# Darkbblue/generic-diffusion-feature

Measured on AMD Instinct MI355X. Metric: images/sec feature-extract, SDXL 1024^2 single-timestep, higher is better.
Workload: dtype f16; 1 GPU; SDXL UNet 1024x1024 (latent 128x128), batch 16/GPU, t=100, hooks=config_xl_practical (4 ids, 15.73 MB/img), full forward; global_batch=16, parallelism=dp1 (batch sharded, weights broadcast once), residual_stream=fp32 master + fp16 shadow, launched_by=single process, max_inflight_forwards=0

## Files before the change

generic-diffusion-feature_amd/csrc/gemm.hip:

```cpp
#include "gemm_mainloop_ring.h"
#include "gemm_mainloop_8phase.h"
#include "gemm_epilogue.h"
#include <cstdio>
#include <cstdlib>
#include <cstring>
#include <deque>
#include <mutex>
#include <string>

namespace gdf {

template <int MODE, int BM, int BN, int STAGES, bool GEGLU, bool DIT, bool BF = false, bool QKN = false, bool SPLIT = false, bool MX = false,
          bool GNS = false>
__device__ __forceinline__ void gemm_body(const GemmParams& p) {
  using T = GemmTile<MODE, BM, BN, STAGES, GEGLU, DIT, BF, QKN, SPLIT, MX, GNS>;
  extern __shared__ __attribute__((aligned(16))) char smem[];
  T t(p, smem);
  const int tiles_n = (p.N + BN - 1) / BN;
  const int nblk = ((p.M + BM - 1) / BM) * tiles_n;
  constexpr bool PERSIST = (STAGES == 8);
  int vb = blockIdx.x;
  do {
  t.locate(vb, tiles_n, nblk);
  f32x4 acc[T::FM][T::FN];
#pragma unroll
  for (int i = 0; i < T::FM; ++i)
#pragma unroll
    for (int j = 0; j < T::FN; ++j) acc[i][j] = f32x4{0.f, 0.f, 0.f, 0.f};
  if constexpr (STAGES == 8) gemm_mainloop_8phase_256(t, acc);
  else if constexpr (STAGES == 9) gemm_mainloop_8phase_320(t, acc);
  else gemm_mainloop_ring(t, acc);
  __syncthreads();
  gemm_epilogue(t, acc);
  if constexpr (!PERSIST) break;
  vb += gridDim.x;
  if (vb >= nblk) break;
  asm volatile("s_waitcnt lgkmcnt(0)" ::: "memory");
  __builtin_amdgcn_s_barrier();
  } while (true);
}

template <int MODE, int BM, int BN, int STAGES, bool GEGLU>
__global__ __launch_bounds__(BM * 2, 2) void gemm_kernel(const GemmParams p) {
  gemm_body<MODE, BM, BN, STAGES, GEGLU, false>(p);
}
template <int MODE, int BM, int BN, int STAGES>
__global__ __launch_bounds__(BM * 2, 2) void gemm_gn_kernel(const GemmParams p) {
  gemm_body<MODE, BM, BN, STAGES, false, false, false, false, false, false, true>(p);
}
template <int MODE, int BM, int BN, int STAGES, bool GEGLU>
__global__ __launch_bounds__(BM * 2, 2) void gemm_split_kernel(const GemmParams p) {
  gemm_body<MODE, BM, BN, STAGES, GEGLU, false, false, false, true>(p);
}
template <int BM, int BN, int STAGES, bool BF, bool QKN>
__global__ __launch_bounds__(BM * 2, 2) void gemm_dit_kernel(const GemmParams p) {
  gemm_body<A_DENSE, BM, BN, STAGES, false, true, BF, QKN>(p);
}

template <int BM, int BN, int STAGES, bool BF, bool QKN>
__global__ __launch_bounds__(BM * 2, 2) void gemm_dit_split_kernel(const GemmParams p) {
  gemm_body<A_DENSE, BM, BN, STAGES, false, true, BF, QKN, true>(p);
}

template <int BM, int BN, int STAGES>
__global__ __launch_bounds__(BM * 2, 2) void gemm_mx_kernel(const GemmParams p) {
  gemm_body<A_DENSE, BM, BN, STAGES, false, true, true, false, false, true>(p);
}

static int persist_wgs() {
  static const int off = [] { const char* e = getenv("GDF_PERSIST"); return e && atoi(e) == 0; }();
  if (off) return 1 << 30;
  static std::atomic<int> cus[16];
  int dev = 0;
  if (hipGetDevice(&dev) != hipSuccess || dev < 0 || dev >= 16) return 1 << 30;
  int n = cus[dev].load(std::memory_order_relaxed);
  if (n == 0) {
    if (hipDeviceGetAttribute(&n, hipDeviceAttributeMultiprocessorCount, dev) != hipSuccess || n < 8 || (n & 7)) n = 1 << 30;
    cus[dev].store(n, std::memory_order_relaxed);
  }
  return n;
}

template <int MODE, int BM, int BN, int STAGES, bool GEGLU, bool DIT = false, bool BF = false, bool QKN = false, bool SPLIT = false, bool MX = false,
          bool GNS = false>
static hipError_t launch_t(const GemmParams& p, hipStream_t s) {
  const int tiles_m = (p.M + BM - 1) / BM, tiles_n = (p.N + BN - 1) / BN;
  const int smem = (STAGES >= 8 ? 2 : STAGES) * (BM * 128 + BN * 128);
  static std::atomic<uint64_t> attr_mask{0};
  {
    const void* fn;
    if constexpr (MX) fn = (const void*)gemm_mx_kernel<BM, BN, STAGES>;
    else if constexpr (GNS) fn = (const void*)gemm_gn_kernel<MODE, BM, BN, STAGES>;
    else if constexpr (DIT && SPLIT) fn = (const void*)gemm_dit_split_kernel<BM, BN, STAGES, BF, QKN>;
    else if constexpr (DIT) fn = (const void*)gemm_dit_kernel<BM, BN, STAGES, BF, QKN>;
    else if constexpr (SPLIT) fn = (const void*)gemm_split_kernel<MODE, BM, BN, STAGES, GEGLU>;
    else fn = (const void*)gemm_kernel<MODE, BM, BN, STAGES, GEGLU>;
    const hipError_t e = ensure_dyn_smem(attr_mask, fn, smem);
    if (e != hipSuccess) return e;
  }
  GemmParams q = p;
  q.sb_gm = q.sb_gn = 0;
  if (!p.no_superblock) {
    const int conc = (p.cus > 0 ? p.cus / 8 : 32) * ((BM == 256) ? 1 : 2);
    for (int gn = 4; gn >= 2; gn >>= 1) {
      const int gm = conc / gn;
      if (tiles_n % gn == 0 && tiles_m % gm == 0 && (tiles_m / gm) * (tiles_n / gn) >= 8 && tiles_n > gn) {
        q.sb_gm = gm; q.sb_gn = gn;
        break;
      }
    }
  }
  int gx = tiles_m * tiles_n;
  const int pw = (p.cus > 0 && p.cus < persist_wgs()) ? p.cus : persist_wgs();
  if (STAGES == 8 && gx > pw && !(p.batch > 1)) gx = pw;
  const dim3 grid(gx, (STAGES == 2 && p.splitk > 1) ? p.splitk : p.batch > 1 ? p.batch : 1);
  if constexpr (MX) hipLaunchKernelGGL((gemm_mx_kernel<BM, BN, STAGES>), grid, dim3(BM * 2), smem, s, q);
  else if constexpr (GNS) hipLaunchKernelGGL((gemm_gn_kernel<MODE, BM, BN, STAGES>), grid, dim3(BM * 2), smem, s, q);
  else if constexpr (DIT && SPLIT) hipLaunchKernelGGL((gemm_dit_split_kernel<BM, BN, STAGES, BF, QKN>), grid, dim3(BM * 2), smem, s, q);
  else if constexpr (DIT) hipLaunchKernelGGL((gemm_dit_kernel<BM, BN, STAGES, BF, QKN>), grid, dim3(BM * 2), smem, s, q);
  else if constexpr (SPLIT) hipLaunchKernelGGL((gemm_split_kernel<MODE, BM, BN, STAGES, GEGLU>), grid, dim3(BM * 2), smem, s, q);
  else hipLaunchKernelGGL((gemm_kernel<MODE, BM, BN, STAGES, GEGLU>), grid, dim3(BM * 2), smem, s, q);
  return hipGetLastError();
}

static double round_fill(long tiles, int slots) {
  if (tiles <= 0) return 0.0;
  const long rounds = (tiles + slots - 1) / slots;
  return (double)tiles / (double)(rounds * slots);
}

static int pick_variant_any(const GemmParams& p);
static bool is_split(const GemmParams& p) { return !p.dit && (p.k_w > 0 || p.o16_lo > 0); }
static bool is_dit_split(const GemmParams& p) { return p.dit && (p.k_w > 0 || p.o16_lo > 0); }
static int pick_variant(const GemmParams& p) {
  const int v = pick_variant_any(p);
  if (is_dit_split(p)) return (v == 8256 || v == 1256) ? 8256 : 128;
  if (!is_split(p) || v == 16) return v;
  if (p.geglu) return v == 825 ? 825 : 128;
  if (p.mode == A_CONV_SMALLC) return v == 160 ? 160 : 128;
  return (v == 932 || v == 160) ? v : 128;
}
static int pick_variant_any(const GemmParams& p) {
  const int S1 = p.cus > 0 ? p.cus : 256, S2 = 2 * S1;
  if (p.dit) {
    const long t256 = (long)((p.M + 255) / 256) * ((p.N + 255) / 256);
    if (p.variant == 128 || p.variant == 1256 || p.variant == 2128 || p.variant == 8256) return p.variant;
    if (t256 >= 128 && (long)((p.N + 255) / 256) * 256 <= (long)p.N + p.N / 8) return 8256;
    return (p.N % 128 == 0 && (long)((p.M + 255) / 256) * (p.N / 128) >= 256) ? 2128 : 128;
  }
  if (p.bn == 16) return 16;
  if (p.splitk > 1) {
    static const int force = [] { const char* e = getenv("GDF_SPLITK_TILE"); return e ? atoi(e) : 0; }();
    if (force == 160 && p.N % 160 == 0) return 160;
    if (force == 128 && p.N % 128 == 0) return 128;
    return (p.N % 160 == 0) ? 160 : 128;
  }
  if (p.variant) return p.variant;
  const long tiles256 = (long)((p.M + 255) / 256) * ((p.N + 127) / 128);
  const long tiles320 = (long)((p.M + 255) / 256) * ((p.N + 319) / 320);
  if (p.geglu) {
    const long tm256 = (p.M + 255) / 256, tm128 = (p.M + 127) / 128;
    double best = 0.0; int bv = 128;
    auto cand = [&](int v, double rate, long tiles, int slots) { const double sc = rate * round_fill(tiles, slots); if (sc > best) { best = sc; bv = v; } };
    if (p.N % 256 == 0) cand(825, 1.00, tm256 * (p.N / 256), S1);
    if (p.N % 320 == 0) cand(320, 0.95, tm256 * (p.N / 320), S1);
    cand(256, 0.80, tm256 * ((p.N + 127) / 128), S1);
    cand(128, 0.70, tm128 * ((p.N + 127) / 128), S2);
    return bv;
  }
  if (p.mode != A_DENSE) {
    if (p.N % 320 == 0) {
      const double s932 = 1.00 * round_fill(tiles320, S1), s160 = 0.85 * round_fill((long)((p.M + 127) / 128) * (p.N / 160), S2);
      const double s128 = 0.70 * round_fill((long)((p.M + 127) / 128) * ((p.N + 127) / 128), S2);
      return (s932 >= s160 && s932 >= s128) ? 932 : (s160 >= s128 ? 160 : 128);
    }
    if (p.N % 160 == 0) return 160;
    if (p.N % 256 == 0 && (long)((p.M + 255) / 256) * (p.N / 256) >= 256) return 826;
    return (p.N <= 128 && p.M >= (1 << 20)) ? 256 : 128;
  }
  if (p.res32 && p.K <= 1536 && p.N % 160 == 0 && tiles320 <= S2 &&
      !(p.N % 320 == 0 && p.N >= 640 && p.K >= 640 && tiles320 % S1 == 0)) return 160;
  if (p.N % 320 == 0) {
    const double s932 = 1.00 * round_fill(tiles320, S1), s160 = 0.87 * round_fill((long)((p.M + 127) / 128) * (p.N / 160), S2);
    const double s128 = 0.72 * round_fill((long)((p.M + 127) / 128) * ((p.N + 127) / 128), S2);
    return (s932 >= s160 && s932 >= s128) ? 932 : (s160 >= s128 ? 160 : 128);
  }
  if (p.N % 160 == 0 && p.K >= 1024) return 160;
  if ((long)p.M * p.N >= (1L << 26) && tiles256 >= S2) return 256;
  return 128;
}

bool gemm_qkn_ok(int M, int N, int K) {
  GemmParams g{}; g.M = M; g.N = N; g.K = K; g.dit = 1; g.mode = A_DENSE;
  const int v = pick_variant(g);
  return v == 8256 || v == 1256;
}

const char* gemm_kernel_name(const GemmParams& p) {
  const int v = pick_variant(p);
  int bm = 128, bn = 128, st = 2;
  if (v == 16) bn = 16; else if (v == 160) bn = 160; else if (v == 256) { bm = 256; st = 3; } else if (v == 320) { bm = 256; bn = 320; }
  else if (v == 825) { bm = 256; bn = 256; st = 8; } else if (v == 932) { bm = 256; bn = 320; st = 9; } else if (v == 826) { bm = 256; bn = 256; st = 8; }
  if (p.mode == A_CONV_SMALLC && v != 160) { bm = 128; bn = 128; st = 2; }
  char tmp[64];
  if (p.gn_partial && !p.dit) snprintf(tmp, sizeof tmp, "gemm_gn_kernel<%d, %d, %d, %d>", p.mode, bm, bn, st);
  else if (p.dit && p.mx) snprintf(tmp, sizeof tmp, "gemm_mx_kernel<256, 256, 8>");
  else if (p.dit) snprintf(tmp, sizeof tmp, "%s<%d, %d, %d, %s, %s>", is_dit_split(p) ? "gemm_dit_split_kernel" : "gemm_dit_kernel", v == 128 ? 128 : 256, (v == 1256 || v == 8256) ? 256 : 128, v == 8256 ? 8 : v == 2128 ? 3 : 2, p.bf16 ? "true" : "false", p.qkn_nq ? "true" : "false");
  else snprintf(tmp, sizeof tmp, "%s<%d, %d, %d, %d, %s>", is_split(p) ? "gemm_split_kernel" : "gemm_kernel", p.mode, bm, bn, st, p.geglu ? "true" : "false");
  static std::mutex mu;
  static std::deque<std::string> names;
  std::lock_guard<std::mutex> lk(mu);
  for (const std::string& n : names) if (n == tmp) return n.c_str();
  names.emplace_back(tmp);
  return names.back().c_str();
}

int gemm_gn_slab_rows(const GemmParams& p) {
  if ((p.mode != A_CONV3 && p.mode != A_CONV_SMALLC) || p.dit || p.geglu || p.splitk > 1 || p.batch > 1 || is_split(p) || p.bn == 16) return 0;
  if ((p.M % 64) != 0 || (p.N % 8) != 0) return 0;
  const int v = pick_variant(p);
  if (p.mode == A_CONV_SMALLC) return v != 160 ? 64 : 0;
  if (v == 932) return (p.M % 128) == 0 ? 128 : 0;
  return (v == 128 || v == 160 || v == 256 || v == 826) ? 64 : 0;
}

hipError_t gemm_check(const GemmParams& p) {
  if (p.mode != A_CONV_SMALLC && (p.K % BK) != 0) return hipErrorInvalidValue;
  if (p.mode == A_CONV3 && (p.Cin % BK) != 0) return hipErrorInvalidValue;
  if (p.k_w > 0 && (p.K != 2 * p.k_w || (p.k_w % BK) != 0 || p.mode == A_CONV_SMALLC || (p.dit && !p.bf16) || (p.mode == A_CONV3 && (p.k_w % (9 * BK)) != 0)))
    return hipErrorInvalidValue;
  if (p.o16_lo > 0 && ((p.dit && !p.bf16) || p.bn == 16 || (p.o16_lo % 8) != 0)) return hipErrorInvalidValue;
  if (p.out_f16 && !(p.dit && p.bf16)) return hipErrorInvalidValue;
  const int v = pick_variant(p);
  if (v != 16 && ((p.geglu ? p.N / 2 : p.N) % 8) != 0) return hipErrorInvalidValue;
  if (p.bf16 && !p.dit) return hipErrorInvalidValue;
  if (p.gn_partial) return (gemm_gn_slab_rows(p) == 0 || !p.out16) ? hipErrorInvalidValue : hipSuccess;
  if (p.dit) {
    if (p.mode != A_DENSE || p.geglu || p.batch > 1) return hipErrorInvalidValue;
    if (p.qkn_nq && ((v != 8256 && v != 1256) || (p.qkn_nq % 128) != 0)) return hipErrorInvalidValue;
    if (p.qkn_nq && (p.res32 || p.res16 || p.rowvec || p.aux16 || p.out32)) return hipErrorInvalidValue;
    if (p.mx && (!p.bf16 || p.qkn_nq || is_dit_split(p) || (p.N % 8))) return hipErrorInvalidValue;
    if (!p.mx && is_dit_split(p) && v != 8256 && p.qkn_nq) return hipErrorInvalidValue;
    return hipSuccess;
  }
  if (p.geglu && (p.mode != A_DENSE || (p.N % 32) != 0)) return hipErrorInvalidValue;
  if (v == 16 && (p.mode == A_CONV_SMALLC || (is_split(p) && !p.geglu && p.mode != A_CONV3))) return hipErrorInvalidValue;
  return hipSuccess;
}

bool gemm_variant_ok(const GemmParams& p) {
  if (!p.variant || p.dit || p.mode == A_CONV_SMALLC) return true;
  const int v = pick_variant(p);
  if (p.geglu) return v != 16 && v != 160 && v != 932 && v != 826;
  if (p.mode == A_DENSE) return v != 825 && v != 826;
  return v != 825;
}

hipError_t launch_gemm(const GemmParams& p, hipStream_t s) {
  if (p.M <= 0 || p.N <= 0) return hipSuccess;
// ... 178 lines not shown
```

generic-diffusion-feature_amd/csrc/gemm_epilogue.h:

```cpp
#pragma once
#include "gemm_tile.h"

namespace gdf {

template <class T>
__device__ __forceinline__ void gemm_epilogue(T& t, f32x4 (&acc)[T::FM][T::FN]) {
  GDF_TILE_GEOMETRY(T);
  GDF_TILE_STATE(t);
  _Float16* const out16 = t.out16;
  const float* const e_res32 = QKN ? nullptr : p.res32;
  const float* const e_rowvec = QKN ? nullptr : p.rowvec;
  const _Float16* const e_res16 = QKN ? nullptr : p.res16;
  _Float16* const e_aux16 = QKN ? nullptr : p.aux16;
  float* const e_out32 = QKN ? nullptr : (STAGES == 2 && p.splitk > 1) ? p.out32 + (size_t)blockIdx.y * p.o32_sstride : p.out32;
  static_assert(!GEGLU || (FN % 2 == 0), "GEGLU needs an even number of column fragments per wave");
  constexpr int FNV = GEGLU ? FN / 2 : FN;
  constexpr int WTNV = FNV * 16;
  constexpr int SLD = WTNV + 4;
  constexpr int PR = (FM * FN >= 32) ? 16 : 32;
  constexpr int PASSES = WTM / PR;
  constexpr int FPP = FM / PASSES;
  float* st = (float*)(smem) + wave * (PR * SLD);
  constexpr int OUTW = WTNV;
  constexpr int LPR = OUTW / 8;
  constexpr int RPI = 64 / LPR;
  constexpr int NIT = (PR + RPI - 1) / RPI;
  const bool lane_ok = lane < RPI * LPR;
  const int Nout = GEGLU ? p.N / 2 : p.N;
  const int ocol0 = GEGLU ? (n0 + wn * WTN) / 2 : (n0 + wn * WTN);
  const int lc = (lane % LPR) * 8;
  const int col = ocol0 + lc;
  const int nv = (col < Nout) ? ((Nout - col >= 8) ? 8 : (Nout - col)) : 0;
  const bool full = nv == 8;

  const float a_sc = p.acc_scale != 0.f ? p.acc_scale : 1.0f;
  const float o_sc = p.out16_scale != 0.f ? p.out16_scale : 1.0f;
  float mxc[8];
#pragma unroll
  for (int e = 0; e < 8; ++e) mxc[e] = 1.f;
  if constexpr (MX) {
    if (full && p.mx_colscale) {
      const f32x4 c0 = *(const f32x4*)(p.mx_colscale + col), c1 = *(const f32x4*)(p.mx_colscale + col + 4);
#pragma unroll
      for (int e = 0; e < 4; ++e) { mxc[e] = c0[e]; mxc[4 + e] = c1[e]; }
    }
  }
  float bv[8];
  float bh[FNV], bgt[FNV];
#pragma unroll
  for (int e = 0; e < 8; ++e) bv[e] = 0.f;
#pragma unroll
  for (int j = 0; j < FNV; ++j) { bh[j] = 0.f; bgt[j] = 0.f; }
  if (p.bias) {
    if (GEGLU) {
#pragma unroll
      for (int j = 0; j < FNV; ++j) {
        const int bcol = n0 + wn * WTN + j * 32 + frow;
        if (bcol + 16 < p.N) { bh[j] = p.bias[bcol]; bgt[j] = p.bias[bcol + 16]; }
      }
    } else if (full) {
      const f32x4 a0 = *(const f32x4*)(p.bias + col), a1 = *(const f32x4*)(p.bias + col + 4);
#pragma unroll
      for (int e = 0; e < 4; ++e) { bv[e] = a0[e]; bv[4 + e] = a1[e]; }
    } else if (BN == 16) {
      for (int e = 0; e < nv; ++e) bv[e] = p.bias[col + e];
    }
  }

  constexpr bool RAGGED = (BN == 16);
  const bool rv_in_opnd = e_rowvec && !e_res32;
  auto sample_of = [&](int row) -> int {
    if (DIT && p.rv_seg_rows > 0 && row >= p.rv_seg_rows) return (row - p.rv_seg_rows) / p.rv_rps2;
    if (DIT && p.rv_tok) return row % p.rows_per_sample;
    return row / p.rows_per_sample;
  };
  float gsum[GNS ? 8 : 1], gsq[GNS ? 8 : 1];
#pragma unroll
  for (int e = 0; e < (GNS ? 8 : 1); ++e) gsum[e] = gsq[e] = 0.f;
#pragma unroll
  for (int ps = 0; ps < PASSES; ++ps) {
    f32x4 opnd[NIT][2];
    int rowi[NIT];
    bool okr[NIT];
#pragma unroll
    for (int it = 0; it < NIT; ++it) {
      const int lrp = it * RPI + lane / LPR;
      rowi[it] = m0 + wm * WTM + ps * PR + lrp;
      okr[it] = (RAGGED ? nv > 0 : full) && lane_ok && lrp < PR && rowi[it] < p.M;
      opnd[it][0] = opnd[it][1] = f32x4{0.f, 0.f, 0.f, 0.f};
    }
    if (!RAGGED) {
      if (e_res32) {
#pragma unroll
        for (int it = 0; it < NIT; ++it)
          if (okr[it]) {
            const f32x4* rp = (const f32x4*)(e_res32 + (size_t)rowi[it] * p.ldres + col);
            opnd[it][0] = rp[0]; opnd[it][1] = rp[1];
          }
      } else if (e_rowvec) {
#pragma unroll
        for (int it = 0; it < NIT; ++it)
          if (okr[it]) {
            const f32x4* rv = (const f32x4*)(e_rowvec + (size_t)sample_of(rowi[it]) * p.ldrv + col);
            opnd[it][0] = rv[0]; opnd[it][1] = rv[1];
          }
      } else if (e_res16) {
#pragma unroll
        for (int it = 0; it < NIT; ++it)
          if (okr[it]) opnd[it][0] = *(const f32x4*)(e_res16 + (size_t)rowi[it] * p.ldres + col);
      }
    }
#pragma unroll
    for (int i2 = 0; i2 < FPP; ++i2)
#pragma unroll
      for (int j = 0; j < FNV; ++j)
        if constexpr (GEGLU) {
#pragma unroll
          for (int r = 0; r < 4; r += 2) {
            const f32x2 hh = {acc[ps * FPP + i2][2 * j][r], acc[ps * FPP + i2][2 * j][r + 1]};
            const f32x2 gg = {acc[ps * FPP + i2][2 * j + 1][r], acc[ps * FPP + i2][2 * j + 1][r + 1]};
            const f32x2 x = (hh + bh[j]) * gelu_erf2(gg + bgt[j]);
            st[(i2 * 16 + fk * 4 + r) * SLD + j * 16 + frow] = x[0];
            st[(i2 * 16 + fk * 4 + r + 1) * SLD + j * 16 + frow] = x[1];
          }
        } else {
#pragma unroll
          for (int r = 0; r < 4; ++r) st[(i2 * 16 + fk * 4 + r) * SLD + j * 16 + frow] = acc[ps * FPP + i2][j][r] * a_sc;
        }
    __builtin_amdgcn_wave_barrier();
    float v[NIT][8];
#pragma unroll
    for (int it = 0; it < NIT; ++it) {
      int lr = it * RPI + lane / LPR;
      if (!(lane_ok && lr < PR)) lr = 0;
      const f32x4 x0 = *(const f32x4*)(st + lr * SLD + lc), x1 = *(const f32x4*)(st + lr * SLD + lc + 4);
      if constexpr (MX) {
        const float rs = (okr[it] && p.mx_rowscale) ? p.mx_rowscale[rowi[it]] : 1.f;
#pragma unroll
        for (int e = 0; e < 4; ++e) { v[it][e] = x0[e] * (rs * mxc[e]) + bv[e]; v[it][4 + e] = x1[e] * (rs * mxc[4 + e]) + bv[4 + e]; }
      } else {
#pragma unroll
        for (int e = 0; e < 4; ++e) { v[it][e] = x0[e] + bv[e]; v[it][4 + e] = x1[e] + bv[4 + e]; }
      }
    }
    if (DIT && p.act == 1) {
#pragma unroll
      for (int it = 0; it < NIT; ++it)
#pragma unroll
        for (int e = 0; e < 8; ++e) v[it][e] = gelu_tanh(v[it][e]);
    }
    if constexpr (DIT && WTN == 128 && QKN) {
      if (p.qkn_nq > 0 && ocol0 < 2 * p.qkn_nq) {
        const float* nw = (ocol0 < p.qkn_nq ? p.qkn_wq : p.qkn_wk) + lc;
        const f32x4 w0 = *(const f32x4*)nw, w1 = *(const f32x4*)(nw + 4);
#pragma unroll
        for (int it = 0; it < NIT; ++it) {
          float ss = 0.f;
#pragma unroll
          for (int e = 0; e < 8; ++e) ss += v[it][e] * v[it][e];
#pragma unroll
          for (int off = 8; off > 0; off >>= 1) ss += __shfl_xor(ss, off);
          const float r = rsqrtf(ss * (1.0f / 128.0f) + p.qkn_eps);
          const int row = rowi[it];
          const int pos = (p.qkn_seg_rows > 0 && row >= p.qkn_seg_rows) ? p.qkn_pos1 + (row - p.qkn_seg_rows) % p.qkn_rps2
                                                                        : p.qkn_pos0 + row % p.qkn_rps;
          f32x4 c0 = {1.f, 1.f, 1.f, 1.f}, c1 = c0, s0 = {0.f, 0.f, 0.f, 0.f}, s1 = s0;
          if (okr[it]) {
            const float* cp = p.rope_cos + (size_t)pos * 128 + lc;
            const float* sp = p.rope_sin + (size_t)pos * 128 + lc;
            c0 = *(const f32x4*)cp; c1 = *(const f32x4*)(cp + 4); s0 = *(const f32x4*)sp; s1 = *(const f32x4*)(sp + 4);
          }
          float t[8];
#pragma unroll
          for (int e = 0; e < 4; ++e) { t[e] = v[it][e] * r * w0[e]; t[4 + e] = v[it][4 + e] * r * w1[e]; }
          v[it][0] = t[0] * c0[0] - t[1] * s0[0]; v[it][1] = t[1] * c0[1] + t[0] * s0[1];
          v[it][2] = t[2] * c0[2] - t[3] * s0[2]; v[it][3] = t[3] * c0[3] + t[2] * s0[3];
          v[it][4] = t[4] * c1[0] - t[5] * s1[0]; v[it][5] = t[5] * c1[1] + t[4] * s1[1];
          v[it][6] = t[6] * c1[2] - t[7] * s1[2]; v[it][7] = t[7] * c1[3] + t[6] * s1[3];
        }
      }
    }
    const bool aux_early = DIT && p.rv_mul && e_aux16;
    if (!RAGGED && aux_early) {
#pragma unroll
      for (int it = 0; it < NIT; ++it)
        if (okr[it]) {
          f16x8 hv;
#pragma unroll
          for (int e = 0; e < 8; ++e) hv[e] = hook16<DIT>(v[it][e]);
          *(f16x8*)(e_aux16 + (size_t)rowi[it] * p.ldaux + col) = hv;
        }
    }
    if (!RAGGED) {
      if (rv_in_opnd) {
        if (DIT && p.rv_mul) {
#pragma unroll
          for (int it = 0; it < NIT; ++it)
#pragma unroll
            for (int e = 0; e < 4; ++e) { v[it][e] *= opnd[it][0][e]; v[it][4 + e] *= opnd[it][1][e]; }
        } else {
#pragma unroll
          for (int it = 0; it < NIT; ++it)
#pragma unroll
            for (int e = 0; e < 4; ++e) { v[it][e] += opnd[it][0][e]; v[it][4 + e] += opnd[it][1][e]; }
        }
      } else if (e_rowvec) {
#pragma unroll
        for (int it = 0; it < NIT; ++it)
          if (okr[it]) {
            const f32x4* rv = (const f32x4*)(e_rowvec + (size_t)sample_of(rowi[it]) * p.ldrv + col);
            if (DIT && p.rv_mul) {
#pragma unroll
              for (int e = 0; e < 4; ++e) { v[it][e] *= rv[0][e]; v[it][4 + e] *= rv[1][e]; }
            } else {
#pragma unroll
              for (int e = 0; e < 4; ++e) { v[it][e] += rv[0][e]; v[it][4 + e] += rv[1][e]; }
            }
          }
      }
      if (e_aux16 && !aux_early) {
#pragma unroll
// ... 107 lines not shown
```

generic-diffusion-feature_amd/csrc/gemm_mainloop_8phase.h:

```cpp
#pragma once
#include "gemm_tile.h"

namespace gdf {

template <class T>
__device__ __forceinline__ void gemm_mainloop_8phase_256(T& t, f32x4 (&acc)[T::FM][T::FN]) {
  GDF_TILE_GEOMETRY(T);
  GDF_TILE_STATE(t);
  GDF_TILE_OPERANDS(t);
  static_assert((MODE == A_DENSE || MODE == A_CONV3) && BM == 256 && (BN == 256 || BN == 320) && FM == 4 && FN == BN / 32, "8-phase schedule: 4x2 waves of 64 x BN/2");
  constexpr int FNH = FN / 2;
  constexpr int BHALF = BN / 2;
  constexpr bool B3 = (BN == 320);
  const bool g1 = wave >= 4;
  auto b_unit_row = [&](int unit, int j) { return (wave >> 2) * 128 + unit * 64 + ((wave & 3) * 2 + j) * 8; };
  uint32_t ha[2][2], hb[2][3];
  uint32_t hm[2][2];
  int hbq[2];
#pragma unroll
  for (int h = 0; h < 2; ++h) {
    const bool big = B3 && (g1 == (h == 1));
    hbq[h] = !B3 ? wave * 2 : (big ? (wave & 3) * 3 : 12 + (wave & 3) * 2);
#pragma unroll
    for (int j = 0; j < 2; ++j) {
      const int m = m0 + h * 128 + (wave * 2 + j) * 8 + lrow;
      if (MODE == A_DENSE) {
        ha[h][j] = (m < p.M) ? (uint32_t)m * (uint32_t)p.lda * 2u + (uint32_t)chunk * 16u : OOB;
        hm[h][j] = 0;
      } else {
        conv_row(m, ha[h][j], hm[h][j]);
      }
    }
#pragma unroll
    for (int j = 0; j < 3; ++j) {
      const int r = (B3 ? h * BHALF + (hbq[h] + j) * 8 : b_unit_row(h, j)) + lrow;
      hb[h][j] = (n0 + r < p.N) ? (uint32_t)(n0 + r) * ldb + (uint32_t)chunk * 16u : OOB;
    }
  }
  auto stage = [&](int kt, int buf, auto which) {
    constexpr int W = decltype(which)::value;
    if constexpr (W < 2) {
      char* base = smem + buf * A_TILE + W * 16384 + wave * 2048;
#pragma unroll
      for (int j = 0; j < 2; ++j) {
        glds16(rsA, base + j * 1024, MODE == A_DENSE ? ha[W][j] + koffA(kt) : conv_off(kt, ha[W][j], hm[W][j]));
      }
    } else {
      constexpr int H = W - 2;
      char* base = smem + 2 * A_TILE + buf * B_TILE + (B3 ? H * (BHALF * 128) + hbq[H] * 1024 : b_unit_row(H, 0) * 128);
#pragma unroll
      for (int j = 0; j < 2; ++j) glds16(rsB, base + j * 1024, hb[H][j] + koffB(kt));
      if (B3 && (g1 == (H == 1))) glds16(rsB, base + 2 * 1024, hb[H][2] + koffB(kt));
    }
  };
  auto wait_tile = [&]() {
    if (B3 && !g1) wait_vmcnt<7>(); else wait_vmcnt<6>();
  };
  constexpr std::integral_constant<int, 0> ALO{};
  constexpr std::integral_constant<int, 1> AHI{};
  constexpr std::integral_constant<int, 2> BLO{};
  constexpr std::integral_constant<int, 3> BHI{};
  f16x8 a8[4][2], b8[FNH][2];
  uint32_t fa[2], fb[2];
#pragma unroll
  for (int kk = 0; kk < 2; ++kk) {
    const int ch = MX ? 2 * fk + kk : kk * 4 + fk;
    fa[kk] = (uint32_t)((wm * WTM + frow) * 128 + ((ch ^ (frow & 7)) << 4));
    fb[kk] = (uint32_t)(2 * A_TILE + (wn * WTN + frow) * 128 + ((ch ^ (frow & 7)) << 4));
    asm volatile("" : "+v"(fa[kk]), "+v"(fb[kk]));
  }
  auto rd_a = [&](const int cur) {
#pragma unroll
    for (int i = 0; i < 4; ++i)
#pragma unroll
      for (int kk = 0; kk < 2; ++kk) a8[i][kk] = *(const f16x8*)(smem + fa[kk] + (cur * A_TILE + i * 2048));
  };
  auto rd_b = [&](const int cur, int half) {
#pragma unroll
    for (int j = 0; j < FNH; ++j)
#pragma unroll
      for (int kk = 0; kk < 2; ++kk) b8[j][kk] = *(const f16x8*)(smem + fb[kk] + (cur * B_TILE + (half * FNH + j) * 2048));
  };
  auto mma_q = [&](auto ah, auto bh) {
    constexpr int AH = decltype(ah)::value, BH = decltype(bh)::value;
    if constexpr (MX) {
#pragma unroll
      for (int i = 0; i < 2; ++i)
#pragma unroll
        for (int jj = 0; jj < FNH; ++jj) {
          const int j = snake(i, jj, FNH);
          acc[AH * 2 + i][BH * FNH + j] = mfma_mx8(a8[AH * 2 + i][0], a8[AH * 2 + i][1], b8[j][0], b8[j][1], acc[AH * 2 + i][BH * FNH + j]);
        }
    } else {
#pragma unroll
      for (int kk = 0; kk < 2; ++kk)
#pragma unroll
        for (int i = 0; i < 2; ++i)
#pragma unroll
          for (int jj = 0; jj < FNH; ++jj) {
            const int j = snake(i + kk, jj, FNH);
            acc[AH * 2 + i][BH * FNH + j] = mfma16<BF>(a8[AH * 2 + i][kk], b8[j][kk], acc[AH * 2 + i][BH * FNH + j]);
          }
    }
  };
  auto bar = [&]() {
    __builtin_amdgcn_sched_barrier(0);
    __builtin_amdgcn_s_barrier();
    __builtin_amdgcn_sched_barrier(0);
  };
  auto lgkm0 = [&]() { asm volatile("s_waitcnt lgkmcnt(0)" ::: "memory"); };
  constexpr std::integral_constant<int, 0> Q0{};
  constexpr std::integral_constant<int, 1> Q1{};

  stage(0, 0, ALO); stage(0, 0, AHI); stage(0, 0, BLO); stage(0, 0, BHI);
  stage(1, 1, ALO); stage(1, 1, AHI); stage(1, 1, BLO);
  wait_tile();
  bar();
  if (g1) bar();
  auto ktile = [&](int kt, const int cur) {
    rd_a(cur); rd_b(cur, 0); stage(kt + 1, cur ^ 1, BHI); lgkm0();
    bar(); mma_q(Q0, Q0); mma_q(Q1, Q0); bar();
    rd_b(cur, 1); stage(kt + 2, cur, ALO); stage(kt + 2, cur, AHI); stage(kt + 2, cur, BLO); wait_tile(); lgkm0();
    bar(); mma_q(Q1, Q1); mma_q(Q0, Q1); bar();
  };
  {
    int kt = 0;
    if constexpr (MODE == A_DENSE) {
      for (; kt + 1 < nk; kt += 2) { ktile(kt, 0); ktile(kt + 1, 1); }
      if (kt < nk) ktile(kt, 0);
    } else {
      for (; kt < nk; ++kt) ktile(kt, kt & 1);
    }
  }
  if (!g1) bar();
  wait_vmcnt<0>();
}

template <class T>
__device__ __forceinline__ void gemm_mainloop_8phase_320(T& t, f32x4 (&acc)[T::FM][T::FN]) {
  GDF_TILE_GEOMETRY(T);
  GDF_TILE_STATE(t);
  GDF_TILE_OPERANDS(t);
  static_assert((MODE == A_DENSE || MODE == A_CONV3) && BM == 256 && BN == 320 && FM == 8 && FN == 5 && WGN == 4,
                "8-phase schedule, 2x4 waves of 128x80");
  uint32_t ua[4];
  uint32_t um[4];
#pragma unroll
  for (int q = 0; q < 4; ++q) {
    const int m = m0 + (wave >> 2) * 128 + q * 32 + (wave & 3) * 8 + lrow;
    if (MODE == A_DENSE) {
      ua[q] = (m < p.M) ? (uint32_t)m * (uint32_t)p.lda * 2u + (uint32_t)chunk * 16u : OOB;
      um[q] = 0;
    } else {
      conv_row(m, ua[q], um[q]);
    }
  }
  uint32_t ub[5];
#pragma unroll
  for (int j = 0; j < 5; ++j) {
    const int qi = j < 3 ? wave * 3 + j : 24 + wave * 2 + (j - 3);
    const int n = n0 + qi * 8 + lrow;
    ub[j] = (n < p.N) ? (uint32_t)n * ldb + (uint32_t)chunk * 16u : OOB;
  }
  auto stage_a = [&](int kt, int buf, int q) {
    char* dst = smem + buf * A_TILE + ((wave >> 2) * 128 + q * 32 + (wave & 3) * 8) * 128;
    glds16(rsA, dst, MODE == A_DENSE ? ua[q] + koffA(kt) : conv_off(kt, ua[q], um[q]));
  };
  auto stage_b = [&](int kt, int buf, auto part) {
    constexpr int PT = decltype(part)::value;
    char* base = smem + 2 * A_TILE + buf * B_TILE;
#pragma unroll
    for (int j = (PT ? 3 : 0); j < (PT ? 5 : 3); ++j) {
      const int qi = j < 3 ? wave * 3 + j : 24 + wave * 2 + (j - 3);
      glds16(rsB, base + qi * 1024, ub[j] + koffB(kt));
    }
  };
  constexpr std::integral_constant<int, 0> B1{};
  constexpr std::integral_constant<int, 1> B2{};
  f16x8 a4[2][2], b10[5][2];
  uint32_t fa[2], fb[2];
#pragma unroll
  for (int kk = 0; kk < 2; ++kk) {
    fa[kk] = (uint32_t)((wm * WTM + frow) * 128 + (((kk * 4 + fk) ^ (frow & 7)) << 4));
    fb[kk] = (uint32_t)(2 * A_TILE + (wn * WTN + frow) * 128 + (((kk * 4 + fk) ^ (frow & 7)) << 4));
    asm volatile("" : "+v"(fa[kk]), "+v"(fb[kk]));
  }
  auto rd_aq = [&](const int cur, int q) {
#pragma unroll
    for (int i = 0; i < 2; ++i)
#pragma unroll
      for (int kk = 0; kk < 2; ++kk) a4[i][kk] = *(const f16x8*)(smem + fa[kk] + (cur * A_TILE + (q * 2 + i) * 2048));
  };
  auto rd_ball = [&](const int cur) {
#pragma unroll
    for (int j = 0; j < 5; ++j)
#pragma unroll
      for (int kk = 0; kk < 2; ++kk) b10[j][kk] = *(const f16x8*)(smem + fb[kk] + (cur * B_TILE + j * 2048));
  };
  auto mma_q = [&](auto qq) {
    constexpr int Q = decltype(qq)::value;
#pragma unroll
    for (int kk = 0; kk < 2; ++kk)
#pragma unroll
      for (int i = 0; i < 2; ++i)
#pragma unroll
        for (int jj = 0; jj < 5; ++jj) {
          const int j = snake(i + kk, jj, 5);
          acc[Q * 2 + i][j] = __builtin_amdgcn_mfma_f32_16x16x32_f16(a4[i][kk], b10[j][kk], acc[Q * 2 + i][j], 0, 0, 0);
        }
  };
  auto bar = [&]() {
    __builtin_amdgcn_sched_barrier(0);
    __builtin_amdgcn_s_barrier();
    __builtin_amdgcn_sched_barrier(0);
  };
  auto lgkm0 = [&]() { asm volatile("s_waitcnt lgkmcnt(0)" ::: "memory"); };
  constexpr std::integral_constant<int, 0> P0{};
  constexpr std::integral_constant<int, 1> P1{};
  constexpr std::integral_constant<int, 2> P2{};
  constexpr std::integral_constant<int, 3> P3{};
  const bool g1 = wave >= 4;

  constexpr bool TWO_PHASE = (MODE == A_DENSE) && !SPLIT;
  stage_b(0, 0, B1); stage_b(0, 0, B2); stage_a(0, 0, 0); stage_a(0, 0, 1); stage_a(0, 0, 2); stage_a(0, 0, 3);
  if constexpr (TWO_PHASE) {
    stage_b(1, 1, B1); stage_a(1, 1, 0); stage_a(1, 1, 1);
    wait_vmcnt<5>();
  } else {
    stage_b(1, 1, B1); stage_b(1, 1, B2); stage_a(1, 1, 0); stage_a(1, 1, 1); stage_a(1, 1, 2);
    wait_vmcnt<8>();
  }
  bar();
  if (g1) bar();
  if constexpr (TWO_PHASE) {
    f16x8 a8[4][2];
    auto rd_ah = [&](const int cur, int h) {
#pragma unroll
      for (int i = 0; i < 4; ++i)
#pragma unroll
        for (int kk = 0; kk < 2; ++kk) a8[i][kk] = *(const f16x8*)(smem + fa[kk] + (cur * A_TILE + (h * 4 + i) * 2048));
    };
    auto mma_h = [&](auto hh) {
      constexpr int H = decltype(hh)::value;
#pragma unroll
      for (int kk = 0; kk < 2; ++kk)
#pragma unroll
        for (int i = 0; i < 4; ++i)
#pragma unroll
          for (int jj = 0; jj < 5; ++jj) {
            const int j = snake(i + kk, jj, 5);
            acc[H * 4 + i][j] = __builtin_amdgcn_mfma_f32_16x16x32_f16(a8[i][kk], b10[j][kk], acc[H * 4 + i][j], 0, 0, 0);
          }
    };
    auto ktile = [&](int kt, const int cur) {
      rd_ball(cur); rd_ah(cur, 0); stage_b(kt + 1, cur ^ 1, B2); stage_a(kt + 1, cur ^ 1, 2); stage_a(kt + 1, cur ^ 1, 3); lgkm0();
      bar(); mma_h(P0); bar();
      rd_ah(cur, 1); stage_b(kt + 2, cur, B1); stage_a(kt + 2, cur, 0); stage_a(kt + 2, cur, 1); wait_vmcnt<5>(); lgkm0();
      bar(); mma_h(P1); bar();
    };
    int kt = 0;
    for (; kt + 1 < nk; kt += 2) { ktile(kt, 0); ktile(kt + 1, 1); }
    if (kt < nk) ktile(kt, 0);
  } else {
    auto ktile4 = [&](int kt, const int cur) {
      rd_ball(cur); rd_aq(cur, 0); stage_a(kt + 1, cur ^ 1, 3); lgkm0();
      bar(); mma_q(P0); bar();
      rd_aq(cur, 1); stage_b(kt + 2, cur, B1); lgkm0();
      bar(); mma_q(P1); bar();
      rd_aq(cur, 2); stage_b(kt + 2, cur, B2); stage_a(kt + 2, cur, 0); lgkm0();
// ... 18 lines not shown
```

generic-diffusion-feature_amd/csrc/gemm_tile.h:

```cpp
#pragma once
#include "gemm_common.h"

namespace gdf {

__device__ __forceinline__ constexpr int snake(int row, int j, int n) { return (row & 1) ? n - 1 - j : j; }

template <int MODE_, int BM_, int BN_, int STAGES_, bool GEGLU_, bool DIT_, bool BF_, bool QKN_, bool SPLIT_, bool MX_, bool GNS_>
struct GemmTile {
  static constexpr int MODE = MODE_, BM = BM_, BN = BN_, STAGES = STAGES_;
  static constexpr bool GEGLU = GEGLU_, DIT = DIT_, BF = BF_, QKN = QKN_, SPLIT = SPLIT_, MX = MX_, GNS = GNS_;
  static_assert(!BF || DIT, "bf16 operands exist on the MMDiT path only");
  static_assert(!GNS || (!DIT && !GEGLU && !SPLIT && !MX && BN >= 128), "GroupNorm partial sums: plain epilogues, one statistics slab per wave tile (WTM rows)");
  static_assert(!MX || (DIT && STAGES == 8 && !SPLIT && !QKN && !GEGLU), "fp8 operands: the 256x256 two-group MMDiT kernel only");
  static constexpr int NW = BM / 32;
  static constexpr int WGN = (BN == 320 && !GEGLU && STAGES != 8) ? 4 : (BN >= 128) ? 2 : 1;
  static constexpr int WGM = NW / WGN;
  static constexpr int WTM = BM / WGM;
  static constexpr int WTN = BN / WGN;
  static constexpr int FM = WTM / 16, FN = WTN / 16;
  static constexpr int A_TILE = BM * 128;
  static constexpr int B_TILE = BN * 128;
  static constexpr int STAGE = A_TILE + B_TILE;
  static constexpr int A_PER_WAVE = BM / 8 / NW;
  static constexpr int B_INSTR = BN / 8;
  static constexpr int B_PER_WAVE = (B_INSTR + NW - 1) / NW;
  static constexpr int LPT = A_PER_WAVE + B_PER_WAVE;
  static_assert(STAGES == 2 || STAGES == 8 || STAGES == 9 || (STAGES == 3 && B_INSTR % NW == 0), "3-stage ring needs a uniform per-wave load count");

  const GemmParams& p;
  char* const smem;
  const int tid, lane, wave;
  int lrow;
  int chunk;
  int wm, wn;
  int frow, fk;
  int vb;
  int m0, n0;
  __amdgpu_buffer_rsrc_t rsA, rsB;
  _Float16* out16;
  uint32_t ldb;
  int nk, kt0, kt1;
  int IH, IW;
  int nkw;
  uint32_t a_lo;
  int cbw;

  __device__ __forceinline__ GemmTile(const GemmParams& p_, char* smem_)
      : p(p_), smem(smem_), tid(threadIdx.x), lane(threadIdx.x & 63), wave(__builtin_amdgcn_readfirstlane(threadIdx.x >> 6)) {}

  __device__ __forceinline__ void locate(int vb_, int tiles_n, int nblk) {
    vb = vb_;
    int tile_m, tile_n;
    if (p.sb_gn > 0) {
      const int conc = p.sb_gm * p.sb_gn;
      const int sbn = tiles_n / p.sb_gn;
      const int nsb = (nblk / conc);
      const int grouped = (nsb >> 3) * 8 * conc;
      int sb, li;
      if (vb < grouped) {
        const int xcd = vb & 7, j = vb >> 3;
        sb = (j / conc) * 8 + xcd; li = j - (j / conc) * conc;
      } else {
        const int t = vb - grouped;
        sb = (nsb >> 3) * 8 + t / conc; li = t - (t / conc) * conc;
      }
      const int sbr = sb / sbn, sbc = sb - sbr * sbn;
      tile_m = sbr * p.sb_gm + li / p.sb_gn;
      tile_n = sbc * p.sb_gn + li % p.sb_gn;
    } else {
      const int t = xcd_remap(vb, nblk);
      tile_m = t / tiles_n; tile_n = t - tile_m * tiles_n;
    }
    m0 = tile_m * BM; n0 = tile_n * BN;
    rsA = __builtin_amdgcn_make_buffer_rsrc((void*)p.A, 0, p.a_bytes, 0x00020000);
    rsB = __builtin_amdgcn_make_buffer_rsrc((void*)(p.Wt + (size_t)blockIdx.y * p.w_bstride), 0, p.w_bytes, 0x00020000);
    out16 = p.out16 ? p.out16 + (size_t)blockIdx.y * p.o_bstride : nullptr;
    lrow = lane >> 3;
    chunk = (lane & 7) ^ lrow;
    ldb = (uint32_t)((SPLIT && p.k_w > 0) ? p.k_w : p.K) * 2u;
    nk = (MODE == A_CONV_SMALLC) ? 2 : p.K / BK;
    kt0 = 0; kt1 = nk;
    if (STAGES == 2 && p.splitk > 1) {
      kt0 = (int)((long)nk * blockIdx.y / p.splitk);
      kt1 = (int)((long)nk * (blockIdx.y + 1) / p.splitk);
    }
    IH = p.ups ? 2 * p.H : p.H; IW = p.ups ? 2 * p.W : p.W;
    nkw = (SPLIT && p.k_w > 0) ? p.k_w / BK : nk;
    a_lo = SPLIT ? p.a_lo_bytes : 0u;
    cbw = nkw / 9;
    wm = wave / WGN; wn = wave - wm * WGN;
    frow = lane & 15; fk = lane >> 4;
  }


  __device__ __forceinline__ uint32_t koffA(int kt) const {
    if constexpr (!SPLIT) return kt < nk ? (uint32_t)kt * 128u : OOB;
    else return kt < nkw ? (uint32_t)kt * 128u : (kt < nk ? a_lo + (uint32_t)(kt - nkw) * 128u : OOB);
  }
  __device__ __forceinline__ uint32_t koffB(int kt) const {
    if constexpr (!SPLIT) return kt < nk ? (uint32_t)kt * 128u : OOB;
    else return kt < nk ? (uint32_t)(kt < nkw ? kt : kt - nkw) * 128u : OOB;
  }
  __device__ __forceinline__ uint32_t chanb(int cbk) const {
    if constexpr (!SPLIT) return (uint32_t)cbk * 128u;
    else return cbk < cbw ? (uint32_t)cbk * 128u : a_lo + (uint32_t)(cbk - cbw) * 128u;
  }
  __device__ __forceinline__ void conv_row(int m, uint32_t& base, uint32_t& mask) const {
    const int hw = p.OH * p.OW;
    const int n = m / hw;
    const int rem = m - n * hw;
    const int oy = rem / p.OW, ox = rem - oy * p.OW;
    const int uy = oy * p.stride - 1 + p.pad0, ux = ox * p.stride - 1 + p.pad0;
    const int by = p.ups ? (uy >> 1) : uy, bx = p.ups ? (ux >> 1) : ux;
    base = (uint32_t)((n * p.H + by) * p.W + bx) * (uint32_t)p.lda * 2u + (uint32_t)chunk * 16u;
    uint32_t mk = 0;
    if (m < p.M) {
#pragma unroll
      for (int tp = 0; tp < 9; ++tp) {
        const int iy = uy + tp / 3, ix = ux + tp % 3;
        if ((iy >= 0) & (iy < IH) & (ix >= 0) & (ix < IW)) mk |= 1u << tp;
      }
    }
    if (p.ups) mk |= ((uint32_t)(uy & 1) << 9) | ((uint32_t)(ux & 1) << 10);
    mask = mk;
  }
  __device__ __forceinline__ uint32_t conv_tap_off(int tp, int cbk, uint32_t base, uint32_t mask, bool live = true) const {
    const int ky = tp / 3, kx = tp - ky * 3;
    const uint32_t rowb = (uint32_t)p.W * (uint32_t)p.lda * 2u, pixb = (uint32_t)p.lda * 2u;
    uint32_t off;
    if (!p.ups) {
      off = base + ((uint32_t)ky * rowb + (uint32_t)kx * pixb + chanb(cbk));
    } else {
      off = base + ((ky == 2 ? rowb : 0u) + (kx == 2 ? pixb : 0u) + chanb(cbk));
      if (ky == 1 && (mask & 512u)) off += rowb;
      if (kx == 1 && (mask & 1024u)) off += pixb;
    }
    const uint32_t bit = live ? (1u << tp) : 0u;
    return (mask & bit) ? off : OOB;
  }
  __device__ __forceinline__ uint32_t conv_off(int kt, uint32_t base, uint32_t mask) const {
    const int cbk = kt / 9;
    return conv_tap_off(kt - cbk * 9, cbk, base, mask, kt < nk);
  };
};

#define GDF_TILE_GEOMETRY(T)                                                                                                                    \
  [[maybe_unused]] constexpr int MODE = T::MODE, BM = T::BM, BN = T::BN, STAGES = T::STAGES;                                                   \
  [[maybe_unused]] constexpr bool GEGLU = T::GEGLU, DIT = T::DIT, BF = T::BF, QKN = T::QKN, SPLIT = T::SPLIT, MX = T::MX, GNS = T::GNS;        \
  [[maybe_unused]] constexpr int NW = T::NW, WGN = T::WGN, WGM = T::WGM, WTM = T::WTM, WTN = T::WTN, FM = T::FM, FN = T::FN;                  \
  [[maybe_unused]] constexpr int A_TILE = T::A_TILE, B_TILE = T::B_TILE, STAGE = T::STAGE, A_PER_WAVE = T::A_PER_WAVE, B_INSTR = T::B_INSTR,   \
                                 B_PER_WAVE = T::B_PER_WAVE, LPT = T::LPT
#define GDF_TILE_STATE(t)                                                                                                                       \
  [[maybe_unused]] const GemmParams& p = t.p;                                                                                                   \
  [[maybe_unused]] char* const smem = t.smem;                                                                                                   \
  [[maybe_unused]] const int lane = t.lane, wave = t.wave, lrow = t.lrow, chunk = t.chunk, wm = t.wm, wn = t.wn, frow = t.frow, fk = t.fk;     \
  [[maybe_unused]] const int vb = t.vb, m0 = t.m0, n0 = t.n0, nk = t.nk, kt0 = t.kt0, kt1 = t.kt1;                                             \
  [[maybe_unused]] const uint32_t ldb = t.ldb;                                                                                                  \
  [[maybe_unused]] const __amdgpu_buffer_rsrc_t rsA = t.rsA, rsB = t.rsB
#define GDF_TILE_OPERANDS(t)                                                                                                                    \
  [[maybe_unused]] auto koffA = [&](int kt) -> uint32_t { return t.koffA(kt); };                                                                \
  [[maybe_unused]] auto koffB = [&](int kt) -> uint32_t { return t.koffB(kt); };                                                                \
  [[maybe_unused]] auto conv_row = [&](int m, uint32_t& base, uint32_t& mask) { t.conv_row(m, base, mask); };                                  \
  [[maybe_unused]] auto conv_tap_off = [&](int tp, int cbk, uint32_t base, uint32_t mask) -> uint32_t { return t.conv_tap_off(tp, cbk, base, mask); }; \
  [[maybe_unused]] auto conv_off = [&](int kt, uint32_t base, uint32_t mask) -> uint32_t { return t.conv_off(kt, base, mask); }

}
```

Before: 139.6 images/s.

## Prefetch next persistent tile's K-tile 0 operands during the 256x256 GEMM epilogue

In the persistent 8-stage 256x256 dense GEMM, the LDS layout is rearranged so that the epilogue staging area sits apart from the buffers for K-tile 0 of A and B. While the epilogue of the current tile runs, the next tile's origin is computed and its first-K-tile loads (plus B of K-tile 1) are issued early. The next mainloop then skips those loads. This hides the prologue load latency between tiles, at the cost of a larger LDS footprint and more complex scheduling barriers. A guard against a zero superblock gm is also added.

```diff
diff --git a/generic-diffusion-feature_amd/csrc/gemm.hip b/generic-diffusion-feature_amd/csrc/gemm.hip
--- a/generic-diffusion-feature_amd/csrc/gemm.hip
+++ b/generic-diffusion-feature_amd/csrc/gemm.hip
@@ -20,21 +20,42 @@
   const int nblk = ((p.M + BM - 1) / BM) * tiles_n;
   constexpr bool PERSIST = (STAGES == 8);
   int vb = blockIdx.x;
+  [[maybe_unused]] bool primed = false;
+  [[maybe_unused]] int m0n = 0, n0n = 0;
+  if constexpr (T::PRIME8) t.tile_origin(vb, tiles_n, nblk, m0n, n0n);
   do {
-  t.locate(vb, tiles_n, nblk);
+  if constexpr (T::PRIME8) {
+    t.vb = vb; t.m0 = m0n; t.n0 = n0n;
+    t.locate_rest();
+  } else {
+    t.locate(vb, tiles_n, nblk);
+  }
   f32x4 acc[T::FM][T::FN];
 #pragma unroll
   for (int i = 0; i < T::FM; ++i)
 #pragma unroll
     for (int j = 0; j < T::FN; ++j) acc[i][j] = f32x4{0.f, 0.f, 0.f, 0.f};
-  if constexpr (STAGES == 8) gemm_mainloop_8phase_256(t, acc);
+  if constexpr (STAGES == 8) gemm_mainloop_8phase_256(t, acc, primed);
   else if constexpr (STAGES == 9) gemm_mainloop_8phase_320(t, acc);
   else gemm_mainloop_ring(t, acc);
   __syncthreads();
-  gemm_epilogue(t, acc);
-  if constexpr (!PERSIST) break;
-  vb += gridDim.x;
-  if (vb >= nblk) break;
+  if constexpr (T::PRIME8) {
+    const bool more = vb + (int)gridDim.x < nblk;
+    gemm_epilogue(t, acc, [&]() {
+      if (more) {
+        t.tile_origin(vb + gridDim.x, tiles_n, nblk, m0n, n0n);
+        gemm_prime8_early(t, m0n, n0n);
+      }
+    });
+    if (!more) break;
+    vb += gridDim.x;
+    primed = true;
+  } else {
+    gemm_epilogue(t, acc, NoPrime{});
+    if constexpr (!PERSIST) break;
+    vb += gridDim.x;
+    if (vb >= nblk) break;
+  }
   asm volatile("s_waitcnt lgkmcnt(0)" ::: "memory");
   __builtin_amdgcn_s_barrier();
   } while (true);
@@ -85,7 +106,8 @@
           bool GNS = false>
 static hipError_t launch_t(const GemmParams& p, hipStream_t s) {
   const int tiles_m = (p.M + BM - 1) / BM, tiles_n = (p.N + BN - 1) / BN;
-  const int smem = (STAGES >= 8 ? 2 : STAGES) * (BM * 128 + BN * 128);
+  using T = GemmTile<MODE, BM, BN, STAGES, GEGLU, DIT, BF, QKN, SPLIT, MX, GNS>;
+  const int smem = STAGES == 8 ? T::SMEM8 : (STAGES >= 8 ? 2 : STAGES) * (BM * 128 + BN * 128);
   static std::atomic<uint64_t> attr_mask{0};
   {
     const void* fn;
@@ -104,7 +126,7 @@
     const int conc = (p.cus > 0 ? p.cus / 8 : 32) * ((BM == 256) ? 1 : 2);
     for (int gn = 4; gn >= 2; gn >>= 1) {
       const int gm = conc / gn;
-      if (tiles_n % gn == 0 && tiles_m % gm == 0 && (tiles_m / gm) * (tiles_n / gn) >= 8 && tiles_n > gn) {
+      if (gm > 0 && tiles_n % gn == 0 && tiles_m % gm == 0 && (tiles_m / gm) * (tiles_n / gn) >= 8 && tiles_n > gn) {
         q.sb_gm = gm; q.sb_gn = gn;
         break;
       }
diff --git a/generic-diffusion-feature_amd/csrc/gemm_epilogue.h b/generic-diffusion-feature_amd/csrc/gemm_epilogue.h
--- a/generic-diffusion-feature_amd/csrc/gemm_epilogue.h
+++ b/generic-diffusion-feature_amd/csrc/gemm_epilogue.h
@@ -3,8 +3,9 @@
 
 namespace gdf {
 
-template <class T>
-__device__ __forceinline__ void gemm_epilogue(T& t, f32x4 (&acc)[T::FM][T::FN]) {
+struct NoPrime {};
+template <class T, class Prime>
+__device__ __forceinline__ void gemm_epilogue(T& t, f32x4 (&acc)[T::FM][T::FN], Prime&& prime) {
   GDF_TILE_GEOMETRY(T);
   GDF_TILE_STATE(t);
   _Float16* const out16 = t.out16;
@@ -20,6 +21,7 @@
   constexpr int PR = (FM * FN >= 32) ? 16 : 32;
   constexpr int PASSES = WTM / PR;
   constexpr int FPP = FM / PASSES;
+  static_assert(STAGES != 8 || NW * PR * SLD * 4 == T::EPI_STG8, "the LDS image of the two-group 256x256 kernel is laid out around this area");
   float* st = (float*)(smem) + wave * (PR * SLD);
   constexpr int OUTW = WTNV;
   constexpr int LPR = OUTW / 8;
@@ -67,6 +69,16 @@
     }
   }
 
+  if constexpr (!std::is_same_v<std::decay_t<Prime>, NoPrime>) {
+#pragma unroll
+    for (int j = 0; j < FNV; ++j) asm volatile("" ::"v"(bh[j]), "v"(bgt[j]));
+#pragma unroll
+    for (int e = 0; e < 8; ++e) asm volatile("" ::"v"(bv[e]));
+    __builtin_amdgcn_sched_barrier(0);
+    prime();
+    __builtin_amdgcn_sched_barrier(0);
+  }
+
   constexpr bool RAGGED = (BN == 16);
   const bool rv_in_opnd = e_rowvec && !e_res32;
   auto sample_of = [&](int row) -> int {
diff --git a/generic-diffusion-feature_amd/csrc/gemm_mainloop_8phase.h b/generic-diffusion-feature_amd/csrc/gemm_mainloop_8phase.h
--- a/generic-diffusion-feature_amd/csrc/gemm_mainloop_8phase.h
+++ b/generic-diffusion-feature_amd/csrc/gemm_mainloop_8phase.h
@@ -3,17 +3,45 @@
 
 namespace gdf {
 
+__device__ __forceinline__ constexpr int b8_unit_row(int wave, int unit, int j) { return (wave >> 2) * 128 + unit * 64 + ((wave & 3) * 2 + j) * 8; }
+
 template <class T>
-__device__ __forceinline__ void gemm_mainloop_8phase_256(T& t, f32x4 (&acc)[T::FM][T::FN]) {
+__device__ __forceinline__ void gemm_prime8_early(const T& t, int m0n, int n0n) {
+  GDF_TILE_GEOMETRY(T);
+  static_assert(T::PRIME8, "early prime: the two-group 256x256 tile with every buffer of K-tile 0 beyond the epilogue staging area");
+  const GemmParams& p = t.p;
+#pragma unroll
+  for (int s = 0; s < 3; ++s) {
+    const int kt = s >> 1, unit = s & 1;
+#pragma unroll
+    for (int j = 0; j < 2; ++j) {
+      const int r = b8_unit_row(t.wave, unit, j);
+      const uint32_t hb = (n0n + r + t.lrow < p.N) ? (uint32_t)(n0n + r + t.lrow) * t.ldb + (uint32_t)t.chunk * 16u : OOB;
+      glds16(t.rsB, t.smem + T::B8_OFF + kt * B_TILE + r * 128, hb + t.koffB(kt));
+    }
+  }
+#pragma unroll
+  for (int h = 0; h < 2; ++h)
+#pragma unroll
+    for (int j = 0; j < 2; ++j) {
+      const int m = m0n + h * 128 + (t.wave * 2 + j) * 8 + t.lrow;
+      const uint32_t ha = (m < p.M) ? (uint32_t)m * (uint32_t)p.lda * 2u + (uint32_t)t.chunk * 16u : OOB;
+      glds16(t.rsA, t.smem + T::A8_OFF0 + h * 16384 + t.wave * 2048 + j * 1024, ha + t.koffA(0));
+    }
+}
+
+template <class T>
+__device__ __forceinline__ void gemm_mainloop_8phase_256(T& t, f32x4 (&acc)[T::FM][T::FN], const bool primed) {
   GDF_TILE_GEOMETRY(T);
   GDF_TILE_STATE(t);
   GDF_TILE_OPERANDS(t);
+  constexpr int A_OFF0 = T::A8_OFF0, A_OFF1 = T::A8_OFF1, B_OFF = T::B8_OFF;
   static_assert((MODE == A_DENSE || MODE == A_CONV3) && BM == 256 && (BN == 256 || BN == 320) && FM == 4 && FN == BN / 32, "8-phase schedule: 4x2 waves of 64 x BN/2");
   constexpr int FNH = FN / 2;
   constexpr int BHALF = BN / 2;
   constexpr bool B3 = (BN == 320);
   const bool g1 = wave >= 4;
-  auto b_unit_row = [&](int unit, int j) { return (wave >> 2) * 128 + unit * 64 + ((wave & 3) * 2 + j) * 8; };
+  auto b_unit_row = [&](int unit, int j) { return b8_unit_row(wave, unit, j); };
   uint32_t ha[2][2], hb[2][3];
   uint32_t hm[2][2];
   int hbq[2];
@@ -40,14 +68,14 @@
   auto stage = [&](int kt, int buf, auto which) {
     constexpr int W = decltype(which)::value;
     if constexpr (W < 2) {
-      char* base = smem + buf * A_TILE + W * 16384 + wave * 2048;
+      char* base = smem + (A_OFF0 + buf * (A_OFF1 - A_OFF0)) + W * 16384 + wave * 2048;
 #pragma unroll
       for (int j = 0; j < 2; ++j) {
         glds16(rsA, base + j * 1024, MODE == A_DENSE ? ha[W][j] + koffA(kt) : conv_off(kt, ha[W][j], hm[W][j]));
       }
     } else {
       constexpr int H = W - 2;
-      char* base = smem + 2 * A_TILE + buf * B_TILE + (B3 ? H * (BHALF * 128) + hbq[H] * 1024 : b_unit_row(H, 0) * 128);
+      char* base = smem + B_OFF + buf * B_TILE + (B3 ? H * (BHALF * 128) + hbq[H] * 1024 : b_unit_row(H, 0) * 128);
 #pragma unroll
       for (int j = 0; j < 2; ++j) glds16(rsB, base + j * 1024, hb[H][j] + koffB(kt));
       if (B3 && (g1 == (H == 1))) glds16(rsB, base + 2 * 1024, hb[H][2] + koffB(kt));
@@ -66,14 +94,14 @@
   for (int kk = 0; kk < 2; ++kk) {
     const int ch = MX ? 2 * fk + kk : kk * 4 + fk;
     fa[kk] = (uint32_t)((wm * WTM + frow) * 128 + ((ch ^ (frow & 7)) << 4));
-    fb[kk] = (uint32_t)(2 * A_TILE + (wn * WTN + frow) * 128 + ((ch ^ (frow & 7)) << 4));
+    fb[kk] = (uint32_t)(B_OFF + (wn * WTN + frow) * 128 + ((ch ^ (frow & 7)) << 4));
     asm volatile("" : "+v"(fa[kk]), "+v"(fb[kk]));
   }
   auto rd_a = [&](const int cur) {
 #pragma unroll
     for (int i = 0; i < 4; ++i)
 #pragma unroll
-      for (int kk = 0; kk < 2; ++kk) a8[i][kk] = *(const f16x8*)(smem + fa[kk] + (cur * A_TILE + i * 2048));
+      for (int kk = 0; kk < 2; ++kk) a8[i][kk] = *(const f16x8*)(smem + fa[kk] + ((A_OFF0 + cur * (A_OFF1 - A_OFF0)) + i * 2048));
   };
   auto rd_b = [&](const int cur, int half) {
 #pragma unroll
@@ -112,9 +140,15 @@
   constexpr std::integral_constant<int, 0> Q0{};
   constexpr std::integral_constant<int, 1> Q1{};
 
-  stage(0, 0, ALO); stage(0, 0, AHI); stage(0, 0, BLO); stage(0, 0, BHI);
-  stage(1, 1, ALO); stage(1, 1, AHI); stage(1, 1, BLO);
-  wait_tile();
+  if constexpr (T::PRIME8) {
+    if (!primed) { stage(0, 0, BLO); stage(0, 0, BHI); stage(1, 1, BLO); stage(0, 0, ALO); stage(0, 0, AHI); }
+    stage(1, 1, ALO); stage(1, 1, AHI);
+    wait_vmcnt<4>();
+  } else {
+    stage(0, 0, ALO); stage(0, 0, AHI); stage(0, 0, BLO); stage(0, 0, BHI);
+    stage(1, 1, ALO); stage(1, 1, AHI); stage(1, 1, BLO);
+    wait_tile();
+  }
   bar();
   if (g1) bar();
   auto ktile = [&](int kt, const int cur) {
diff --git a/generic-diffusion-feature_amd/csrc/gemm_tile.h b/generic-diffusion-feature_amd/csrc/gemm_tile.h
--- a/generic-diffusion-feature_amd/csrc/gemm_tile.h
+++ b/generic-diffusion-feature_amd/csrc/gemm_tile.h
@@ -26,6 +26,12 @@
   static constexpr int B_PER_WAVE = (B_INSTR + NW - 1) / NW;
   static constexpr int LPT = A_PER_WAVE + B_PER_WAVE;
   static_assert(STAGES == 2 || STAGES == 8 || STAGES == 9 || (STAGES == 3 && B_INSTR % NW == 0), "3-stage ring needs a uniform per-wave load count");
+  static constexpr int EPI_STG8 = NW * 16 * ((GEGLU ? WTN / 2 : WTN) + 4) * 4;
+  static constexpr bool PRIME8 = STAGES == 8 && MODE == A_DENSE && BN == 256 && EPI_STG8 <= A_TILE + 2048;
+  static constexpr int A8_OFF0 = PRIME8 ? EPI_STG8 : 0, A8_OFF1 = PRIME8 ? 0 : A_TILE;
+  static constexpr int B8_OFF = PRIME8 ? A8_OFF0 + A_TILE : 2 * A_TILE;
+  static constexpr int SMEM8 = B8_OFF + 2 * B_TILE;
+  static_assert(!PRIME8 || (EPI_STG8 % 1024 == 0 && A8_OFF0 >= EPI_STG8 && SMEM8 <= 160 * 1024), "two-group 256x256 LDS image");
 
   const GemmParams& p;
   char* const smem;
@@ -50,6 +56,10 @@
 
   __device__ __forceinline__ void locate(int vb_, int tiles_n, int nblk) {
     vb = vb_;
+    tile_origin(vb_, tiles_n, nblk, m0, n0);
+    locate_rest();
+  }
+  __device__ __forceinline__ void tile_origin(int vb, int tiles_n, int nblk, int& m0_, int& n0_) const {
     int tile_m, tile_n;
     if (p.sb_gn > 0) {
       const int conc = p.sb_gm * p.sb_gn;
@@ -71,7 +81,9 @@
       const int t = xcd_remap(vb, nblk);
       tile_m = t / tiles_n; tile_n = t - tile_m * tiles_n;
     }
-    m0 = tile_m * BM; n0 = tile_n * BN;
+    m0_ = tile_m * BM; n0_ = tile_n * BN;
+  }
+  __device__ __forceinline__ void locate_rest() {
     rsA = __builtin_amdgcn_make_buffer_rsrc((void*)p.A, 0, p.a_bytes, 0x00020000);
     rsB = __builtin_amdgcn_make_buffer_rsrc((void*)(p.Wt + (size_t)blockIdx.y * p.w_bstride), 0, p.w_bytes, 0x00020000);
     out16 = p.out16 ? p.out16 + (size_t)blockIdx.y * p.o_bstride : nullptr;
```

Result: no change. 139.8 images/s, median of 6 (+0.1%).
